# lehduong/Knowledge-Distillation-by-Replacing-Cheap-Conv

Measured on AMD Instinct MI355X. Metric: images/sec KD train step, DeepLabV3+(WRN38) student 1024x2048, higher is better.
Workload: dtype bf16; 1 GPU; KD train step (teacher fwd + student fwd + CE/KD/hint criteria + hint bwd + RAdam), DeepLabV3+(WRN-38) student P92, 1024x2048, 8 img/GPU, random init, teacher through the HIP engine; plan=P92, mode=A, arch=deeplab, hint_loss=mse, per_gpu_batch=8, global_batch=8, parallelism=dp1, teacher_backend=hip, ranks_seen=1

## Files before the change

include/kdcc.h:

```cpp
#ifndef KDCC_H
#define KDCC_H

#include <stddef.h>
#include <stdint.h>

#ifdef __cplusplus
extern "C" {
#endif

typedef void *kd_stream_t;

enum { KD_F32 = 0, KD_BF16 = 1 };
enum {
    KD_OK = 0,
    KD_ERR_INVALID = -1,
    KD_ERR_UNSUPPORTED = -2,
    KD_ERR_WORKSPACE = -3,
    KD_ERR_HIP = -4
};

int kd_version(void);
const char *kd_last_error(void);

typedef struct kd_conv_desc {
    int32_t dtype;
    int32_t N, H, W, Cin;
    int32_t Ho, Wo, Cout;
    int32_t kh, kw, stride, pad, dil;
    int32_t ldx;
} kd_conv_desc;

typedef struct kd_conv_epilogue {
    const void *res_pre;  int32_t ld_res_pre;
    const void *mask;     int32_t ld_mask;     const float *mask_scale;
    const void *res_post; int32_t ld_res_post;
    void *out_raw;        int32_t ld_raw;      int32_t raw_f32;
    void *out_act;        int32_t ld_act;      const float *act_scale; const float *act_shift; int32_t act_relu;
    float *bn_sums;
    const void *cls_w;    float *cls_out;      int32_t ld_cls;      int32_t ncls;
} kd_conv_epilogue;
int32_t kd_conv2d_cls_supported(const kd_conv_desc *d, const kd_conv_epilogue *ep);

int kd_conv2d_fwd(const kd_conv_desc *d, const void *x, const void *w_packed,
                  const kd_conv_epilogue *ep, kd_stream_t stream);
int32_t kd_conv2d_bn_sums_rows(const kd_conv_desc *d, const kd_conv_epilogue *ep);
size_t kd_bn_sums_finish_workspace(int32_t rows, int32_t C);
int kd_bn_sums_finish(const float *part, int32_t rows, int32_t C, float *s1, float *s2, void *workspace, size_t workspace_bytes,
                      kd_stream_t stream);

int32_t kd_conv1x1_dual_supported(const kd_conv_desc *d, int32_t Cin2, int32_t ldx2, const kd_conv_epilogue *ep);
int kd_conv1x1_dual_fwd(const kd_conv_desc *d, const void *x, const void *x2, int32_t Cin2, int32_t ldx2, const void *w_cat,
                        const kd_conv_epilogue *ep, kd_stream_t stream);

int kd_conv_set_persist_cus(int32_t n);

enum { KD_PACK_FWD = 0, KD_PACK_DGRAD = 1 };
int kd_pack_conv_weight(const float *src, void *dst, int32_t dtype, int32_t mode,
                        int32_t Cout, int32_t Cin, int32_t kh, int32_t kw, int32_t cin_pad,
                        kd_stream_t stream);

size_t kd_pw_wgrad_workspace(int32_t M, int32_t Cin, int32_t Cout);
int kd_pw_wgrad(int32_t dtype, int32_t M, int32_t Cin, int32_t Cout,
                const void *a, int32_t lda, const void *dy, int32_t ldy,
                float *dw, int32_t accumulate, void *workspace, size_t workspace_bytes,
                kd_stream_t stream);

size_t kd_conv2d_wgrad_workspace(const kd_conv_desc *d);
int kd_conv2d_wgrad(const kd_conv_desc *d, const void *x, const void *dy, int32_t ld_dy, float *dw,
                    int32_t accumulate, void *workspace, size_t workspace_bytes, kd_stream_t stream);

typedef struct kd_dw_desc {
    int32_t dtype;
    int32_t N, H, W, C;
    int32_t k, pad, dil;
    int32_t ldx, ldy;
} kd_dw_desc;
typedef struct kd_dw_epilogue {
    const void *res_pre;  int32_t ld_res_pre;
    const void *mask;     int32_t ld_mask;     const float *mask_scale;
    const void *res_post; int32_t ld_res_post;
} kd_dw_epilogue;
int kd_pack_dw_weight(const float *src , float *dst ,
                      int32_t C, int32_t k, int32_t flip, kd_stream_t stream);
int kd_dwconv_fwd(const kd_dw_desc *d, const void *x, const float *w_taps, const float *bias,
                  const kd_dw_epilogue *ep, void *y, kd_stream_t stream);
int kd_dwconv_fwd_sum(const kd_dw_desc *d, int32_t n, const void *const *xs, const float *const *w_taps, void *y,
                      kd_stream_t stream);
int kd_dwconv_fwd_fanout(const kd_dw_desc *d, int32_t n, const void *x, const float *const *w_taps, void *const *ys,
                         kd_stream_t stream);
size_t kd_dwconv_wgrad_workspace(const kd_dw_desc *d);
int kd_dwconv_wgrad(const kd_dw_desc *d, const void *x, const void *dy, int32_t ld_dy,
                    float *dw, int32_t accumulate, void *workspace, size_t workspace_bytes,
                    kd_stream_t stream);
size_t kd_dwconv_wgrad_multi_workspace(const kd_dw_desc *d, int32_t n);
int kd_dwconv_wgrad_multi(const kd_dw_desc *d, int32_t n, const void *x, const void *const *dys, int32_t ld_dy,
                          float *const *dws, int32_t accumulate, void *workspace, size_t workspace_bytes,
                          kd_stream_t stream);

int64_t kd_lattice_rows(int32_t N, int32_t H, int32_t W, int32_t dil);
int32_t kd_dwconv_lattice_ok(const kd_dw_desc *d, int32_t n);
int kd_lattice_rows_move(int32_t dtype, int32_t N, int32_t H, int32_t W, int32_t C, int32_t dil, void *img, int32_t ld_img,
                         void *rows, int32_t ld_rows, int32_t to_rows, kd_stream_t stream);
int kd_dwconv_fwd_fanout_lattice(const kd_dw_desc *d, int32_t n, const void *x, const float *const *w_taps, void *const *ys,
                                 kd_stream_t stream);
int kd_dwconv_fwd_sum_lattice(const kd_dw_desc *d, int32_t n, const void *const *xs, const float *const *w_taps, void *y,
                              kd_stream_t stream);
int kd_dwconv_wgrad_multi_lattice(const kd_dw_desc *d, int32_t n, const void *x, const void *const *dys, float *const *dws,
                                  int32_t accumulate, void *workspace, size_t workspace_bytes ,
                                  kd_stream_t stream);

int kd_stem_conv(int32_t dtype, const float *x_nchw, const float *w, void *y,
                 int32_t N, int32_t H, int32_t W, kd_stream_t stream);
int kd_stem_conv_pool(const float *x_nchw, const float *w, void *y_raw, void *y_act, const float *scale,
                      const float *shift, int32_t N, int32_t H, int32_t W, kd_stream_t stream);

int kd_maxpool3x3s2(int32_t dtype, const void *x, int32_t ldx, void *y_raw, int32_t ld_raw,
                    void *y_act, int32_t ld_act, const float *scale, const float *shift,
                    int32_t N, int32_t H, int32_t W, int32_t C, kd_stream_t stream);

int kd_upsample_bilinear_ac(const void *x, int32_t x_dtype, int32_t ldx, void *y, int32_t y_dtype, int32_t ldy,
                            int32_t N, int32_t H, int32_t W, int32_t C, int32_t Ho, int32_t Wo,
                            kd_stream_t stream);

int kd_upsample_bilinear(const void *x, int32_t x_dtype, int32_t ldx, void *y, int32_t y_dtype, int32_t ldy,
                         int32_t N, int32_t H, int32_t W, int32_t C, int32_t Ho, int32_t Wo, int32_t align_corners,
                         kd_stream_t stream);

size_t kd_aspp_image_pool_workspace(int32_t N, int32_t Cin, int32_t Cout);
int kd_aspp_image_pool(int32_t dtype, const void *x, int32_t ldx, const float *w, const float *scale,
                       const float *shift, void *y, int32_t ldy, int32_t N, int32_t H, int32_t W,
                       int32_t Cin, int32_t Cout, void *workspace, size_t workspace_bytes, kd_stream_t stream);
int kd_aspp_image_pool_sums(int32_t dtype, const float *part, const float *w, const float *scale, const float *shift, void *y,
                            int32_t ldy, int32_t N, int32_t H, int32_t W, int32_t Cin, int32_t Cout, void *workspace,
                            size_t workspace_bytes, kd_stream_t stream);

size_t kd_stem_wgrad_workspace(int32_t N, int32_t H, int32_t W);
int kd_stem_wgrad(int32_t dtype, const float *x_nchw, const void *dy, int32_t ld_dy, float *dw, int32_t N, int32_t H,
                  int32_t W, int32_t accumulate, void *workspace, size_t workspace_bytes, kd_stream_t stream);
size_t kd_maxpool3x3s2_bwd_workspace(int32_t N, int32_t H, int32_t W, int32_t C);
int kd_maxpool3x3s2_bwd(int32_t dtype, const void *x, int32_t ldx, const void *gy, int32_t ldgy, void *gx, int32_t ldgx,
                        int32_t N, int32_t H, int32_t W, int32_t C, void *workspace, size_t workspace_bytes,
                        kd_stream_t stream);
size_t kd_upsample_bilinear_ac_bwd_workspace(int32_t N, int32_t H, int32_t W, int32_t C, int32_t Ho, int32_t Wo);
int kd_upsample_bilinear_ac_bwd(const void *gy, int32_t gy_dtype, int32_t ldgy, void *gx, int32_t gx_dtype, int32_t ldgx,
                                int32_t N, int32_t H, int32_t W, int32_t C, int32_t Ho, int32_t Wo,
                                void *workspace, size_t workspace_bytes, kd_stream_t stream);
int kd_upsample_bilinear_bwd(const void *gy, int32_t gy_dtype, int32_t ldgy, void *gx, int32_t gx_dtype, int32_t ldgx,
                             int32_t N, int32_t H, int32_t W, int32_t C, int32_t Ho, int32_t Wo, int32_t align_corners,
// ... 219 lines not shown
```

knowledge-distillation-by-replacing-cheap-conv_amd/_lib.py:

```python
import ctypes as C
import os

_HERE = os.path.dirname(os.path.abspath(__file__))
_sel = os.environ.get("KDCC_LIB", "")
LIB_PATH = (os.path.join(_HERE, "libkdcc_hip_tuning.so") if _sel == "tuning" else _sel if _sel.endswith(".so")
            else os.path.join(_HERE, "libkdcc_hip.so"))


def build_tuning():
    import subprocess
    subprocess.check_call(["make", "-s", "-j", str(min(8, os.cpu_count() or 1)), "-C", os.path.join(_HERE, "csrc"), "TUNING=1"])

KD_F32, KD_BF16 = 0, 1
KD_PACK_FWD, KD_PACK_DGRAD = 0, 1
KD_ERR_UNSUPPORTED = -2
KD_OPT_SGD, KD_OPT_ADAM, KD_OPT_ADAMW_REF = 0, 1, 2
KD_OPT_FIRST, KD_OPT_NESTEROV, KD_OPT_AMSGRAD, KD_OPT_MAXIMIZE = 1, 2, 4, 8

c_int, c_i64, c_f, c_vp, c_sz = C.c_int32, C.c_int64, C.c_float, C.c_void_p, C.c_size_t


class ConvDesc(C.Structure):
    _fields_ = [(n, c_int) for n in ("dtype", "N", "H", "W", "Cin", "Ho", "Wo", "Cout", "kh", "kw", "stride", "pad",
                                     "dil", "ldx")]


class ConvEpilogue(C.Structure):
    _fields_ = [("res_pre", c_vp), ("ld_res_pre", c_int),
                ("mask", c_vp), ("ld_mask", c_int), ("mask_scale", c_vp),
                ("res_post", c_vp), ("ld_res_post", c_int),
                ("out_raw", c_vp), ("ld_raw", c_int), ("raw_f32", c_int),
                ("out_act", c_vp), ("ld_act", c_int), ("act_scale", c_vp), ("act_shift", c_vp), ("act_relu", c_int),
                ("bn_sums", c_vp),
                ("cls_w", c_vp), ("cls_out", c_vp), ("ld_cls", c_int), ("ncls", c_int)]


class DwDesc(C.Structure):
    _fields_ = [(n, c_int) for n in ("dtype", "N", "H", "W", "C", "k", "pad", "dil", "ldx", "ldy")]


class RadamTensor(C.Structure):
    _fields_ = [("p", c_vp), ("g", c_vp), ("exp_avg", c_vp), ("exp_avg_sq", c_vp), ("n", c_i64), ("step", c_int),
                ("lr", c_f), ("beta1", c_f), ("beta2", c_f), ("eps", c_f), ("weight_decay", c_f)]


class OptimTensor(C.Structure):
    _fields_ = [("p", c_vp), ("g", c_vp), ("state", c_vp * 3), ("n", c_i64), ("step", c_i64), ("flags", c_int), ("reserved", c_int),
                ("lr", C.c_double), ("weight_decay", C.c_double), ("eps", C.c_double), ("momentum", C.c_double),
                ("dampening", C.c_double), ("beta1", C.c_double), ("beta2", C.c_double), ("warmup", C.c_double)]


class DwEpilogue(C.Structure):
    _fields_ = [("res_pre", c_vp), ("ld_res_pre", c_int), ("mask", c_vp), ("ld_mask", c_int), ("mask_scale", c_vp),
                ("res_post", c_vp), ("ld_res_post", c_int)]


class DConvDesc(C.Structure):
    _fields_ = [(n, c_int) for n in ("N", "C", "H", "W", "K", "kh", "kw", "stride", "pad", "dil", "groups")]


class View3(C.Structure):
    _fields_ = [("ptr", c_vp), ("dtype", c_int), ("sN", c_i64), ("sC", c_i64), ("sP", c_i64)]


class HrView(C.Structure):
    _fields_ = [("ptr", c_vp), ("H", c_int), ("W", c_int), ("ld", c_int)]


KD_MULTI_MAX = 16


class MultiTargets(C.Structure):
    _fields_ = [("n", c_int), ("t", View3 * KD_MULTI_MAX), ("w", c_f * KD_MULTI_MAX)]


_P = C.POINTER
_SIGS = {
    "kd_version": (c_int, []),
    "kd_last_error": (C.c_char_p, []),
    "kd_conv2d_fwd": (c_int, [_P(ConvDesc), c_vp, c_vp, _P(ConvEpilogue), c_vp]),
    "kd_conv1x1_dual_supported": (c_int, [_P(ConvDesc), c_int, c_int, _P(ConvEpilogue)]),
    "kd_conv1x1_dual_fwd": (c_int, [_P(ConvDesc), c_vp, c_vp, c_int, c_int, c_vp, _P(ConvEpilogue), c_vp]),
    "kd_conv_set_persist_cus": (c_int, [c_int]),
    "kd_conv2d_bn_sums_rows": (c_int, [_P(ConvDesc), _P(ConvEpilogue)]),
    "kd_conv2d_cls_supported": (c_int, [_P(ConvDesc), _P(ConvEpilogue)]),
    "kd_bn_sums_finish_workspace": (c_sz, [c_int, c_int]),
    "kd_bn_sums_finish": (c_int, [c_vp, c_int, c_int, c_vp, c_vp, c_vp, c_sz, c_vp]),
    "kd_pack_conv_weight": (c_int, [c_vp, c_vp, c_int, c_int, c_int, c_int, c_int, c_int, c_int, c_vp]),
    "kd_pw_wgrad_workspace": (c_sz, [c_int, c_int, c_int]),
    "kd_pw_wgrad": (c_int, [c_int, c_int, c_int, c_int, c_vp, c_int, c_vp, c_int, c_vp, c_int, c_vp, c_sz, c_vp]),
    "kd_conv2d_wgrad_workspace": (c_sz, [_P(ConvDesc)]),
    "kd_conv2d_wgrad": (c_int, [_P(ConvDesc), c_vp, c_vp, c_int, c_vp, c_int, c_vp, c_sz, c_vp]),
    "kd_stem_wgrad_workspace": (c_sz, [c_int, c_int, c_int]),
    "kd_stem_wgrad": (c_int, [c_int, c_vp, c_vp, c_int, c_vp, c_int, c_int, c_int, c_int, c_vp, c_sz, c_vp]),
    "kd_maxpool3x3s2_bwd_workspace": (c_sz, [c_int, c_int, c_int, c_int]),
    "kd_maxpool3x3s2_bwd": (c_int, [c_int, c_vp, c_int, c_vp, c_int, c_vp, c_int, c_int, c_int, c_int, c_int, c_vp, c_sz, c_vp]),
    "kd_upsample_bilinear_ac_bwd_workspace": (c_sz, [c_int] * 6),
    "kd_upsample_bilinear_ac_bwd": (c_int, [c_vp, c_int, c_int, c_vp, c_int, c_int, c_int, c_int, c_int, c_int, c_int, c_int, c_vp,
                                            c_sz, c_vp]),
    "kd_zero_insert": (c_int, [c_int, c_vp, c_int, c_vp, c_int, c_int, c_int, c_int, c_int, c_int, c_int, c_int, c_vp]),
    "kd_relu_bn_bwd": (c_int, [c_int, c_vp, c_int, c_vp, c_int, c_vp, c_vp, c_int, c_vp, c_int, c_i64, c_int, c_vp]),
    "kd_channel_sums_workspace": (c_sz, [c_int, c_i64, c_int]),
    "kd_channel_sums": (c_int, [c_int, c_vp, c_int, c_vp, c_int, c_vp, c_int, c_int, c_i64, c_int, c_vp, c_vp, c_vp, c_sz, c_vp]),
    "kd_bn_eval_param_grads": (c_int, [c_vp, c_vp, c_vp, c_vp, c_vp, c_vp, c_vp, c_int, c_int, c_vp]),
    "kd_broadcast_add": (c_int, [c_int, c_vp, c_vp, c_int, c_int, c_i64, c_int, c_f, c_int, c_vp]),
    "kd_conv2d_direct_fwd": (c_int, [_P(DConvDesc), c_vp, c_vp, c_vp, c_vp, c_vp]),
    "kd_conv2d_direct_dgrad": (c_int, [_P(DConvDesc), c_vp, c_vp, c_vp, c_vp]),
    "kd_conv2d_direct_wgrad": (c_int, [_P(DConvDesc), c_vp, c_vp, c_vp, c_vp, c_int, c_vp]),
    "kd_bn2d_fwd": (c_int, [c_vp, c_vp, c_vp, c_vp, c_vp, c_vp, c_vp, c_vp, c_f, c_f, c_int, c_int, c_int, c_int, c_int, c_vp]),
    "kd_bn2d_bwd": (c_int, [c_vp, c_vp, c_vp, c_vp, c_vp, c_vp, c_vp, c_vp, c_vp, c_int, c_int, c_int, c_int, c_int, c_int, c_vp]),
    "kd_bn_nhwc_workspace": (c_sz, [c_i64, c_int]),
    "kd_bn_nhwc_fwd": (c_int, [c_vp, c_int, c_vp, c_int, c_i64, c_int, c_vp, c_vp, c_vp, c_vp, c_vp, c_vp, c_f, c_f, c_int, c_int,
                               c_vp, c_sz, c_vp]),
    "kd_bn_nhwc_bwd": (c_int, [c_vp, c_int, c_vp, c_int, c_vp, c_int, c_vp, c_int, c_vp, c_int, c_i64, c_int, c_vp, c_vp, c_vp, c_vp,
                               c_vp, c_int, c_int, c_int, c_vp, c_sz, c_vp]),
    "kd_bn_nhwc_stats": (c_int, [c_vp, c_int, c_i64, c_int, c_vp, c_vp, c_vp, c_f, c_vp, c_sz, c_vp]),
    "kd_bn_nhwc_apply": (c_int, [c_vp, c_int, c_vp, c_int, c_i64, c_int, c_vp, c_vp, c_vp, c_vp, c_vp, c_vp, c_vp, c_f, c_int, c_vp]),
    "kd_avgpool2x2_nhwc": (c_int, [c_vp, c_int, c_vp, c_int, c_int, c_int, c_int, c_int, c_vp]),
    "kd_avgpool2x2_nhwc_bwd": (c_int, [c_vp, c_int, c_vp, c_int, c_int, c_int, c_int, c_int, c_vp]),
    "kd_pack_dw_weight": (c_int, [c_vp, c_vp, c_int, c_int, c_int, c_vp]),
    "kd_dwconv_fwd": (c_int, [_P(DwDesc), c_vp, c_vp, c_vp, _P(DwEpilogue), c_vp, c_vp]),
    "kd_dwconv_fwd_sum": (c_int, [_P(DwDesc), c_int, c_vp, c_vp, c_vp, c_vp]),
    "kd_dwconv_fwd_fanout": (c_int, [_P(DwDesc), c_int, c_vp, c_vp, c_vp, c_vp]),
    "kd_dwconv_wgrad_workspace": (c_sz, [_P(DwDesc)]),
    "kd_dwconv_wgrad": (c_int, [_P(DwDesc), c_vp, c_vp, c_int, c_vp, c_int, c_vp, c_sz, c_vp]),
    "kd_dwconv_wgrad_multi_workspace": (c_sz, [_P(DwDesc), c_int]),
    "kd_dwconv_wgrad_multi": (c_int, [_P(DwDesc), c_int, c_vp, c_vp, c_int, c_vp, c_int, c_vp, c_sz, c_vp]),
    "kd_lattice_rows": (c_i64, [c_int, c_int, c_int, c_int]),
    "kd_dwconv_lattice_ok": (c_int, [_P(DwDesc), c_int]),
    "kd_lattice_rows_move": (c_int, [c_int, c_int, c_int, c_int, c_int, c_int, c_vp, c_int, c_vp, c_int, c_int, c_vp]),
    "kd_dwconv_fwd_fanout_lattice": (c_int, [_P(DwDesc), c_int, c_vp, c_vp, c_vp, c_vp]),
    "kd_dwconv_fwd_sum_lattice": (c_int, [_P(DwDesc), c_int, c_vp, c_vp, c_vp, c_vp]),
    "kd_dwconv_wgrad_multi_lattice": (c_int, [_P(DwDesc), c_int, c_vp, c_vp, c_vp, c_int, c_vp, c_sz, c_vp]),
    "kd_stem_conv": (c_int, [c_int, c_vp, c_vp, c_vp, c_int, c_int, c_int, c_vp]),
    "kd_scale_by_device_scalar": (c_int, [c_vp, c_int, c_i64, c_vp, c_vp]),
    "kd_pointwise_small": (c_int, [c_vp, c_int, c_vp, c_vp, c_vp, c_int, c_i64, c_int, c_int, c_vp]),
    "kd_conv3x3_small": (c_int, [c_vp, c_int, c_vp, c_vp, c_vp, c_int, c_vp, c_int, c_int, c_int, c_int, c_int, c_int, c_vp]),
    "kd_stem_conv_pool": (c_int, [c_vp, c_vp, c_vp, c_vp, c_vp, c_vp, c_int, c_int, c_int, c_vp]),
    "kd_maxpool3x3s2": (c_int, [c_int, c_vp, c_int, c_vp, c_int, c_vp, c_int, c_vp, c_vp, c_int, c_int, c_int, c_int, c_vp]),
    "kd_upsample_bilinear_ac": (c_int, [c_vp, c_int, c_int, c_vp, c_int, c_int, c_int, c_int, c_int, c_int, c_int, c_int, c_vp]),
    "kd_upsample_bilinear": (c_int, [c_vp, c_int, c_int, c_vp, c_int, c_int, c_int, c_int, c_int, c_int, c_int, c_int, c_int, c_vp]),
    "kd_gated_conv": (c_int, [c_int, c_vp, c_int, c_vp, c_int, c_vp, c_vp, c_int, c_i64, c_int, c_vp]),
    "kd_edge_attention": (c_int, [c_int, c_vp, c_int, c_vp, c_vp, c_vp, c_i64, c_vp]),
    "kd_edge_aspp": (c_int, [c_int, c_vp, c_int, c_int, c_vp, c_vp, c_vp, c_vp, c_int, c_int, c_int, c_int, c_int, c_vp]),
    "kd_canny_workspace": (c_sz, [c_int, c_int, c_int]),
    "kd_canny": (c_int, [c_vp, c_int, c_int, c_int, c_int, c_int, c_int, c_vp, c_vp, c_vp, c_sz, c_vp]),
    "kd_canny_continue": (c_int, [c_int, c_int, c_int, c_int, c_vp, c_vp, c_vp, c_sz, c_vp]),
    "kd_aspp_image_pool_workspace": (c_sz, [c_int, c_int, c_int]),
    "kd_aspp_image_pool": (c_int, [c_int, c_vp, c_int, c_vp, c_vp, c_vp, c_vp, c_int, c_int, c_int, c_int, c_int, c_int,
                                   c_vp, c_sz, c_vp]),
    "kd_aspp_image_pool_sums": (c_int, [c_int, c_vp, c_vp, c_vp, c_vp, c_vp, c_int, c_int, c_int, c_int, c_int, c_int, c_vp, c_sz, c_vp]),
    "kd_bn_fold": (c_int, [c_vp, c_vp, c_vp, c_vp, c_f, c_vp, c_vp, c_int, c_vp]),
    "kd_copy_cast": (c_int, [c_vp, c_int, c_i64, c_i64, c_i64, c_vp, c_int, c_i64, c_i64, c_i64, c_int, c_int, c_i64, c_vp]),
    "kd_loss_workspace": (c_sz, [c_int, c_int, c_i64]),
    "kd_kldiv": (c_int, [_P(View3), _P(View3), c_f, c_int, c_int, c_i64, c_vp, _P(View3), c_f, c_vp, c_sz, c_vp]),
    "kd_hint_mse": (c_int, [_P(View3), _P(View3), c_f, c_int, c_int, c_i64, c_vp, _P(View3), c_f, c_vp, c_sz, c_vp]),
    "kd_weighted_hint_mse": (c_int, [_P(View3), _P(View3), c_vp, c_int, c_int, c_int, c_i64, c_vp, _P(View3), c_f, c_vp,
                                     c_sz, c_vp]),
    "kd_ce2d": (c_int, [_P(View3), c_vp, c_int, c_int, c_int, c_i64, c_vp, c_vp, c_sz, c_vp]),
    "kd_ce2d_up": (c_int, [c_vp, c_vp, c_int, c_int, c_int, c_int, c_int, c_int, c_int, c_int, c_vp, c_vp, c_sz, c_vp]),
    "kd_kldiv_up": (c_int, [c_vp, c_vp, c_f, c_int, c_int, c_int, c_int, c_int, c_int, c_int, c_vp, c_vp, c_sz, c_vp]),
    "kd_logit_metrics_up": (c_int, [c_vp, c_vp, c_vp, c_int, c_int, c_int, c_int, c_int, c_int, c_int, c_int, c_vp, c_vp, c_vp, c_int,
                                    c_vp, c_sz, c_vp]),
    "kd_ce2d_grad": (c_int, [_P(View3), c_vp, c_int, c_int, c_int, c_i64, _P(View3), c_f, c_vp, c_sz, c_vp]),
    "kd_ce2d_weighted": (c_int, [_P(View3), c_vp, c_vp, c_int, c_int, c_int, c_int, c_i64, c_vp, c_vp, c_sz, c_vp]),
    "kd_ce2d_weighted_grad": (c_int, [_P(View3), c_vp, c_vp, c_int, c_int, c_int, c_int, c_i64, _P(View3), c_f, c_vp, c_sz, c_vp]),
    "kd_jsdiv": (c_int, [_P(View3), _P(View3), c_f, c_int, c_int, c_i64, c_vp, _P(View3), c_f, c_vp, c_sz, c_vp]),
    "kd_jsdiv_up": (c_int, [c_vp, c_vp, c_f, c_int, c_int, c_int, c_int, c_int, c_int, c_int, c_vp, c_vp, c_sz, c_vp]),
    "kd_ensemble_kldiv": (c_int, [_P(View3), _P(View3), c_int, c_int, c_i64, c_vp, _P(View3), c_f, c_vp, c_sz, c_vp]),
    "kd_kldiv_multi": (c_int, [_P(View3), _P(MultiTargets), c_f, c_vp, c_int, c_f, c_f, c_int, c_int, c_i64, c_vp, _P(View3), c_vp, c_sz, c_vp]),
    "kd_softmax_mean": (c_int, [_P(MultiTargets), c_f, c_int, c_int, c_i64, _P(View3), c_vp]),
    "kd_focal": (c_int, [_P(View3), c_vp, c_vp, c_f, c_int, c_int, c_int, c_int, c_i64, c_vp, c_vp, c_vp, c_vp, c_vp, c_sz, c_vp]),
    "kd_focal_grad": (c_int, [_P(View3), c_vp, c_vp, c_f, c_int, c_int, c_int, c_int, c_i64, c_vp, c_vp, c_vp, c_vp, _P(View3), c_vp]),
# ... 94 lines not shown
```

knowledge-distillation-by-replacing-cheap-conv_amd/engine.py:

```python
import itertools
import os

import torch
from torch import nn

from . import ops
from ._lib import KD_PACK_DGRAD, KD_PACK_FWD
from .lazy import LazyLogits
from .models.students.transform_blocks import DepthwiseSeparableBlock, GateLayer, RandomMask2d
from .models.wider_resnet import IdentityResidualBlock

_SMALL_CONV = os.environ.get("KDCC_SMALL_CONV", "1") != "0"
_SPLIT_DEC_DGRAD = os.environ.get("KDCC_SPLIT_DEC_DGRAD", "1") != "0"
_STEM_POOL = os.environ.get("KDCC_STEM_POOL", "1") != "0"
_DW_SUM = os.environ.get("KDCC_DW_SUM", "1") != "0"
_CONV_DUAL = os.environ.get("KDCC_CONV_DUAL", "1") != "0"
_FUSE_BN_SUMS = os.environ.get("KDCC_FUSE_BN_SUMS", "1") != "0"
_FUSE_GAP = os.environ.get("KDCC_FUSE_GAP", "1") != "0"


class EngineError(RuntimeError):
    pass


_FOLD_SERIAL = itertools.count(1)


def _is_trainable(mod):
    return any(p.requires_grad for p in mod.parameters())


def _bn_of(bn_seq):
    return bn_seq[0] if isinstance(bn_seq, nn.Sequential) else bn_seq


def _gate_split(mod):
    if isinstance(mod, nn.Sequential) and len(mod) == 2 and isinstance(mod[1], GateLayer):
        return mod[0], mod[1]
    return mod, None


def _is_masked(mod):
    return (isinstance(mod, nn.Sequential) and len(mod) == 3 and isinstance(mod[0], nn.Conv2d) and isinstance(mod[1], RandomMask2d)
            and isinstance(mod[2], nn.Conv2d))


def _act_gate(bn_seq):
    if isinstance(bn_seq, nn.Sequential) and len(bn_seq) > 1:
        return _gate_split(bn_seq[1])[1]
    return None


class _Site:

    def __init__(self, name, mod):
        mod, self.gate = _gate_split(mod)
        self.name, self.mod = name, mod
        self.cheap = isinstance(mod, DepthwiseSeparableBlock)
        self.masked = _is_masked(mod)
        if self.masked:
            self._init_masked(name, mod)
            return
        if self.cheap and self.gate is not None:
            raise EngineError(f"{name}: a gate behind a cheap-conv block is not supported (gates rank the TEACHER's filters)")
        if not self.cheap and not isinstance(mod, nn.Conv2d):
            raise EngineError(f"{name}: unsupported module {type(mod).__name__} in the student graph")
        conv = mod.pointwise_conv if self.cheap else mod
        self.cout = conv.out_channels
        self.cin = (mod.separable_conv if self.cheap else conv).in_channels
        if self.cheap:
            self.k, self.pad, self.dil = mod.geometry
            self.stride = 1
            if mod.separable_conv.bias is not None or mod.pointwise_conv.bias is not None:
                raise EngineError(f"{name}: biased cheap conv inside the fused graph is not supported")
        else:
            if conv.bias is not None or conv.groups != 1:
                raise EngineError(f"{name}: only bias-free dense convs are supported")
            self.k, self.pad, self.dil, self.stride = conv.kernel_size[0], conv.padding[0], conv.dilation[0], conv.stride[0]
        self.trainable = _is_trainable(mod) or (self.gate is not None and self.gate.weight.requires_grad)

    def _init_masked(self, name, mod):
        conv, mask, pw = mod[0], mod[1], mod[2]
        if self.gate is not None:
            raise EngineError(f"{name}: a gate behind a masked site is not supported")
        if conv.bias is not None or conv.groups != 1 or _is_trainable(conv):
            raise EngineError(f"{name}: the conv in front of a RandomMask2d must be a frozen, bias-free dense conv")
        if pw.bias is not None or pw.kernel_size != (1, 1) or pw.stride != (1, 1) or pw.padding != (0, 0) or pw.groups != 1 or \
                pw.in_channels != conv.out_channels or mask.in_channels != conv.out_channels:
            raise EngineError(f"{name}: the conv behind a RandomMask2d must be a bias-free 1x1 over the masked channels")
        self.cin, self.cout = conv.in_channels, pw.out_channels
        self.k, self.pad, self.dil, self.stride = conv.kernel_size[0], conv.padding[0], conv.dilation[0], conv.stride[0]
        self.trainable = pw.weight.requires_grad


class StudentEngine:
    def __init__(self, net, dtype=torch.bfloat16):
        self.net = net
        self.dtype = dtype
        self.hint_names = []
        self._pack = {}
# ... 940 lines not shown
        if gate is not None:
            s2 = s2 / gate.weight.detach().float()
            if gate.weight.requires_grad and grads is not None:
                gbuf = self._grad_like(gate.weight)
                gbuf.copy_(s2)
                grads[gate.weight] = gbuf
                self._grad_done(gate.weight)
        self.probe_grads[name] = s2

    def _conv_wgrad(self, conv, a_in, g, grads, cin=None, cin_rot=0, gate=None):
        w = conv.weight
        if not w.requires_grad:
            return
        if cin is not None and cin != a_in.shape[3]:
            a_in = a_in[..., :cin]
        gw = self._grad_like(w)
        if cin_rot:
            tmp = torch.empty_like(gw)
            ops.conv2d_wgrad(a_in, g, tmp, conv.stride[0], conv.padding[0], conv.dilation[0])
            k = w.shape[1] - cin_rot
            gw[:, cin_rot:].copy_(tmp[:, :k])
            gw[:, :cin_rot].copy_(tmp[:, k:])
        else:
            ops.conv2d_wgrad(a_in, g, gw, conv.stride[0], conv.padding[0], conv.dilation[0])
        if gate is not None:
            gw.mul_(gate.weight.detach().float().view(-1, 1, 1, 1))
        grads[w] = gw
        self._grad_done(w)

    def _wants_bn_sums(self, bn_seq, gate=None):
        bn = _bn_of(bn_seq)
        return bn.weight.requires_grad or bn.bias.requires_grad or (gate is not None and gate.weight.requires_grad)

    def _bn_param_grads(self, bn_seq, g_x, act, grads, sub=None, gate=None, sums=None):
        bn = _bn_of(bn_seq)
        want_gate = gate is not None and gate.weight.requires_grad
        if not (bn.weight.requires_grad or bn.bias.requires_grad or want_gate):
            return
        scale, _ = self._bn_fold(bn_seq)
        s1, s2 = sums if sums is not None else ops.channel_sums(g_x, sub=sub, a=act)
        if gate is not None:
            gv = gate.weight.detach().float()
            if want_gate:
                gbuf = self._grad_like(gate.weight)
                gbuf.copy_(torch.where(scale != 0, s2 / (scale * gv * gv), torch.zeros_like(s2)))
                grads[gate.weight] = gbuf
                self._grad_done(gate.weight)
            s2 = s2 / gv
        if bn.weight.requires_grad or bn.bias.requires_grad:
            self._bn_grads_from_sums(bn, scale, s1, s2, grads)

    def _bn_grads_from_sums(self, bn, scale, s1, s2, grads):
        dg, db = self._grad_like(bn.weight), self._grad_like(bn.bias)
        ops.bn_eval_param_grads(s1.contiguous(), s2.contiguous(), scale, bn.weight.detach().float().contiguous(),
                                bn.bias.detach().float().contiguous(), dg, db)
        for p, gbuf in ((bn.weight, dg), (bn.bias, db)):
            if p.requires_grad:
                grads[p] = gbuf
                self._grad_done(p)

    def _dense_dgrad(self, site, g, in_hw=None, **ep):
        conv = site.mod
        N, H, W, _ = g.shape
        if site.stride != 1:
            if in_hw is None:
                raise EngineError(f"{site.name}: strided input gradient needs the input size")
            g = ops.zero_insert(g, site.stride, in_hw)
            H, W = in_hw
        out = self._new(N, H, W, conv.in_channels)
        ops.conv2d(g, self._w_dgrad(conv, gate=site.gate), 1, site.dil * (site.k - 1) - site.pad, site.dil, out_raw=out, **ep)
        return out

    def _cheap_bwd(self, site, a_in, mid, g, grads, need_in, defer=None, **ep):
        dw, pw = site.mod.separable_conv, site.mod.pointwise_conv
        if pw.weight.requires_grad:
            gw = self._grad_like(pw.weight)
            ops.pw_wgrad(mid, g, gw)
            grads[pw.weight] = gw
            self._grad_done(pw.weight)
        if not (dw.weight.requires_grad or need_in):
            return None
        N, H, W, _ = g.shape
        g_mid = self._new(N, H, W, pw.in_channels)
        ops.conv2d(g, self._w_dgrad(pw), out_raw=g_mid)
        if dw.weight.requires_grad and defer is None:
            gw = self._grad_like(dw.weight)
            ops.dwconv_wgrad(a_in, g_mid, gw, site.k, site.pad, site.dil)
            grads[dw.weight] = gw
            self._grad_done(dw.weight)
        if defer is not None:
            defer.append((g_mid, self._w_dw(dw, True) if need_in else None, site, dw.weight if dw.weight.requires_grad else None))
            return None
        if not need_in:
            return None
        return ops.dwconv(g_mid, self._w_dw(dw, True), site.k, site.dil * (site.k - 1) - site.pad, site.dil, **ep)

    def _site_bwd(self, site, a_in, mid, g, grads, need_in, **ep):
        if site.cheap:
            return self._cheap_bwd(site, a_in, mid, g, grads, need_in, **ep)
        if site.masked:
            return self._masked_bwd(site, mid, g, grads, need_in)
        self._conv_wgrad(site.mod, a_in, g, grads, gate=site.gate)
        if not need_in:
            return None
        return self._dense_dgrad(site, g, in_hw=(a_in.shape[1], a_in.shape[2]), **ep)

    def _block_bwd(self, bi, rec, g_out, g_site_hint, grads):
        blk, sites = rec["blk"], rec["sites"]
        bns = {n: m for n, m in blk.convs.named_children() if n.startswith("bn")}
        g = g_out
        for i in range(len(sites) - 1, -1, -1):
            site, a_in, need_in = sites[i], rec["a_in"][i], rec["rg_a"][i]
            g_in = None
            bn_seq = bns[f"bn{i + 1}"] if i > 0 else blk.bn1
            act_gate = _act_gate(bn_seq) if i > 0 else None
            if g is not None and i in rec.get("probe", {}):
                self._probe(site.name, g, *rec["probe"][i], gate=site.gate, grads=grads)
            if g is not None and (need_in or site.trainable):
                sc, _ = self._act_fold(bn_seq, act_gate)
                ep = dict(mask=a_in, mask_scale=sc)
                sub = None
                if i > 0:
                    sub = g_site_hint.get((bi, i - 1))
                    ep["res_post"] = sub
                elif g_out is not None:
                    if rec["proj"]:
                        psite = _Site(f"{rec['name']}.proj_conv", blk.proj_conv)
                        self._conv_wgrad(blk.proj_conv, a_in, g_out, grads)
                        dual_bwd = (need_in and site.k == 1 and site.stride == 1 and g_out.is_contiguous() and g.is_contiguous() and
                                    self._dual_ok(g.shape, site.cout, g_out.shape[3], site.cin, 1, site.mod, blk.proj_conv, site))
                        if need_in and not dual_bwd:
                            ep["res_pre"] = self._dense_dgrad(psite, g_out, in_hw=(a_in.shape[1], a_in.shape[2]))
                    elif rec["rg_in"]:
                        sub = g_out
                        ep["res_post"] = g_out
                fused = []
                if _FUSE_BN_SUMS and need_in and not site.cheap and self._wants_bn_sums(bn_seq, act_gate):
                    ep["bn_sums"] = fused
                if i == 0 and g_out is not None and rec["proj"] and dual_bwd:
                    self._conv_wgrad(site.mod, a_in, g, grads, gate=site.gate)
                    g_in = self._new(g.shape[0], g.shape[1], g.shape[2], site.cin)
                    try:
                        ops.conv2d(g, self._w_cat(site.mod, blk.proj_conv, "dgrad"), out_raw=g_in, x2=g_out, **ep)
                    except ops.DualUnsupported:
                        if ep.get("bn_sums") is not None:
                            del ep["bn_sums"][:]
                        ep["res_pre"] = self._dense_dgrad(psite, g_out, in_hw=(a_in.shape[1], a_in.shape[2]))
                        g_in = self._dense_dgrad(site, g, in_hw=(a_in.shape[1], a_in.shape[2]), **ep)
                else:
                    g_in = self._site_bwd(site, a_in, rec["mid"][i], g, grads, need_in, **ep)
                if g_in is not None:
                    self._bn_param_grads(bn_seq, g_in, a_in, grads, sub=sub, gate=act_gate, sums=fused[0] if fused else None)
            elif i == 0 and g is None and g_out is not None:
                if rec["proj"]:
                    self._conv_wgrad(blk.proj_conv, a_in, g_out, grads)
                    if need_in:
                        psite = _Site(f"{rec['name']}.proj_conv", blk.proj_conv)
                        sc, _ = self._bn_fold(blk.bn1)
                        g_in = self._dense_dgrad(psite, g_out, in_hw=(a_in.shape[1], a_in.shape[2]), mask=a_in, mask_scale=sc)
                        self._bn_param_grads(blk.bn1, g_in, a_in, grads)
                elif rec["rg_in"]:
                    g_in = g_out
            if i > 0:
                if g_in is None:
                    g_in = g_site_hint.get((bi, i - 1)) if rec["rg_a"][i] else None
                g = g_in
            else:
# ... 282 lines not shown
```

knowledge-distillation-by-replacing-cheap-conv_amd/ops.py:

```python
import ctypes as C
import os

import torch

from . import _lib
from ._lib import (KD_BF16, KD_F32, KD_PACK_DGRAD, KD_PACK_FWD, ConvDesc, ConvEpilogue, DConvDesc, DwDesc, DwEpilogue, MultiTargets, View3,
                   check)


PROFILER = None


def _prof_start():
    if PROFILER is None:
        return None
    e0 = torch.cuda.Event(enable_timing=True)
    e0.record()
    return e0


def _prof_stop(e0, family, work, label, kernel=None):
    if e0 is None or PROFILER is None:
        return
    e1 = torch.cuda.Event(enable_timing=True)
# ... 155 lines not shown
        check(_lib.lib().kd_conv1x1_dual_fwd(C.byref(d), _ptr(x), _ptr(x2), Cin2, ld2, _ptr(w_packed), C.byref(ep), stream_ptr()), "kd_conv1x1_dual_fwd")
    else:
        check(_lib.lib().kd_conv2d_fwd(C.byref(d), _ptr(x), _ptr(w_packed), C.byref(ep), stream_ptr()), "kd_conv2d_fwd")
    if out_rows > 0:
        out_sums.append(opart)
    if prof is not None:
        e1 = torch.cuda.Event(enable_timing=True)
        e1.record()
        epi = "".join(c for c, t in (("p", res_pre), ("m", mask), ("q", res_post), ("r", out_raw), ("a", out_act), ("c", cls_out)) if t is not None)
        prof.append(("conv_igemm", 2.0 * N * Ho * Wo * (algo_cout or Cout) * kh * kw * (algo_cin or (Cin + Cin2)), e0, e1,
                     f"{kh}x{kw} s{stride} d{dil} {H}x{W} {Cin}{'+%d' % Cin2 if Cin2 else ''}->{Cout} [{epi}{'s' if sums_rows or out_rows else ''}]", _lib.last_kernel()))
    if sums_rows > 0:
        s12 = torch.empty((2, Cout), dtype=torch.float32, device=x.device)
        need = _lib.lib().kd_bn_sums_finish_workspace(sums_rows, Cout)
        ws = _ws(need, x.device) if need else None
        check(_lib.lib().kd_bn_sums_finish(_ptr(part), sums_rows, Cout, _ptr(s12[0]), _ptr(s12[1]), _ptr(ws), need, stream_ptr()),
              "kd_bn_sums_finish")
        bn_sums.append((s12[0], s12[1]))
    return out_raw, out_act


def conv_cls_ok(x, Cout, k=3, dil=1):
    if not x.is_cuda or x.dtype != torch.bfloat16 or os.environ.get("KDCC_FUSE_CLS", "1") == "0":
        return False
    N, H, W, Cin = x.shape
    d = ConvDesc(dt_of(x), N, H, W, Cin, H, W, Cout, k, k, 1, dil * (k // 2), dil, nhwc_ld(x))
    ep = ConvEpilogue()
    ep.cls_w, ep.cls_out, ep.ld_cls, ep.ncls = C.c_void_p(256), C.c_void_p(256), 32, 19
    return bool(_lib.lib().kd_conv2d_cls_supported(C.byref(d), C.byref(ep)))


def conv1x1_dual_ok(x, x2, Cout, operands=0):
    if x2 is None or not x.is_cuda or x.dtype != torch.bfloat16 or x2.dtype != x.dtype or tuple(x2.shape[:3]) != tuple(x.shape[:3]):
        return False
    N, H, W, Cin = x.shape
    d = ConvDesc(dt_of(x), N, H, W, Cin, H, W, Cout, 1, 1, 1, 0, 1, nhwc_ld(x))
    ep = ConvEpilogue()
    some = C.c_void_p(x.data_ptr())
    if operands >= 1:
        ep.mask, ep.ld_mask = some, Cout
    if operands >= 2:
        ep.res_post, ep.ld_res_post = some, Cout
    if operands >= 3:
        ep.res_pre, ep.ld_res_pre = some, Cout
    ep.out_raw, ep.ld_raw = some, Cout
    return bool(_lib.lib().kd_conv1x1_dual_supported(C.byref(d), x2.shape[3], nhwc_ld(x2), C.byref(ep)))


def conv1x1_dual_ok_dims(N, H, W, Cin, Cin2, Cout, dtype, operands=0):
    if dtype != torch.bfloat16:
        return False
    d = ConvDesc(KD_BF16, N, H, W, Cin, H, W, Cout, 1, 1, 1, 0, 1, Cin)
    ep = ConvEpilogue()
    if operands >= 1:
        ep.mask, ep.ld_mask = C.c_void_p(256), Cout
    if operands >= 2:
        ep.res_post, ep.ld_res_post = C.c_void_p(256), Cout
    if operands >= 3:
        ep.res_pre, ep.ld_res_pre = C.c_void_p(256), Cout
    ep.out_raw, ep.ld_raw = C.c_void_p(256), Cout
    return bool(_lib.lib().kd_conv1x1_dual_supported(C.byref(d), Cin2, Cin2, C.byref(ep)))


def pw_wgrad(a, dy, dw, accumulate=False, workspace=None):
    _need_cuda(a, dy, dw)
    N, H, W, Cin = a.shape
    Cout = dy.shape[3]
    if tuple(dy.shape[:3]) != (N, H, W) or a.dtype != dy.dtype:
        raise ValueError("pw_wgrad: a / dy mismatch")
    if dw.dtype != torch.float32 or dw.numel() != Cout * Cin or not dw.is_contiguous():
        raise ValueError("pw_wgrad: dw must be contiguous fp32 (Cout,Cin,1,1)")
    M = N * H * W
    need = _lib.lib().kd_pw_wgrad_workspace(M, Cin, Cout)
    if workspace is None or workspace.numel() * workspace.element_size() < need:
        workspace = torch.empty(need, dtype=torch.uint8, device=a.device)
    e0 = _prof_start()
    check(_lib.lib().kd_pw_wgrad(dt_of(a), M, Cin, Cout, _ptr(a), nhwc_ld(a), _ptr(dy), nhwc_ld(dy), _ptr(dw),
                                 int(accumulate), _ptr(workspace), workspace.numel() * workspace.element_size(),
                                 stream_ptr()), "kd_pw_wgrad")
    _prof_stop(e0, "pw_wgrad", 2.0 * M * Cin * Cout, f"pw wgrad {H}x{W} {Cin}->{Cout}")
    return dw


def conv2d_wgrad(x, dy, dw, stride=1, pad=0, dil=1, accumulate=False, workspace=None):
    _need_cuda(x, dy, dw)
    N, H, W, Cin = x.shape
    Cout, Cin_w, kh, kw = dw.shape
    Ho, Wo = conv_out_size(H, kh, stride, pad, dil), conv_out_size(W, kw, stride, pad, dil)
    if Cin_w != Cin or tuple(dy.shape) != (N, Ho, Wo, Cout) or dy.dtype != x.dtype:
        raise ValueError(f"conv2d_wgrad: x {tuple(x.shape)} / dy {tuple(dy.shape)} / dw {tuple(dw.shape)} mismatch")
    if dw.dtype != torch.float32 or not dw.is_contiguous():
        raise ValueError("conv2d_wgrad: dw must be contiguous fp32 (Cout,Cin,kh,kw)")
    d = ConvDesc(dt_of(x), N, H, W, Cin, Ho, Wo, Cout, kh, kw, stride, pad, dil, nhwc_ld(x))
    need = _lib.lib().kd_conv2d_wgrad_workspace(C.byref(d))
    if workspace is None or workspace.numel() * workspace.element_size() < need:
        workspace = torch.empty(need, dtype=torch.uint8, device=x.device)
    prof = PROFILER
    if prof is not None:
        e0 = torch.cuda.Event(enable_timing=True)
        e0.record()
    check(_lib.lib().kd_conv2d_wgrad(C.byref(d), _ptr(x), _ptr(dy), nhwc_ld(dy), _ptr(dw), int(accumulate), _ptr(workspace),
                                     workspace.numel() * workspace.element_size(), stream_ptr()), "kd_conv2d_wgrad")
    if prof is not None:
        e1 = torch.cuda.Event(enable_timing=True)
        e1.record()
        prof.append(("conv_wgrad", 2.0 * N * Ho * Wo * Cout * kh * kw * Cin, e0, e1,
                     f"wgrad {kh}x{kw} s{stride} d{dil} {H}x{W} {Cin}->{Cout}", _lib.last_kernel()))
    return dw


def pack_dw_weight(w, flip=False):
    _need_cuda(w)
    w = w.detach().contiguous().float()
    Cc, one, k, k2 = w.shape
    if one != 1 or k != k2:
        raise ValueError("pack_dw_weight: expected (C,1,k,k)")
    out = torch.empty((k * k, Cc), dtype=torch.float32, device=w.device)
    check(_lib.lib().kd_pack_dw_weight(_ptr(w), _ptr(out), Cc, k, int(flip), stream_ptr()), "kd_pack_dw_weight")
    return out


def _dw_desc(x, k, pad, dil, y=None):
    N, H, W, Cc = x.shape
    return DwDesc(dt_of(x), N, H, W, Cc, k, pad, dil, nhwc_ld(x), nhwc_ld(y) if y is not None else Cc)


def _dw_taps(who, w_taps, k, Cc):
    for w in w_taps:
        if tuple(w.shape) != (k * k, Cc) or w.dtype != torch.float32 or not w.is_contiguous():
            raise ValueError(f"{who}: w_taps must be contiguous fp32 [k*k][C]")


def _dw_grads(who, dws, k, Cc):
    for dw in dws:
        if dw.dtype != torch.float32 or dw.numel() != Cc * k * k or not dw.is_contiguous():
            raise ValueError(f"{who}: dw must be contiguous fp32 (C,1,k,k)")


def _dw_out(who, out, shape, like):
    if out is None:
        out = torch.empty(shape, dtype=like.dtype, device=like.device)
    if tuple(out.shape) != tuple(shape) or out.dtype != like.dtype:
        raise ValueError(f"{who}: bad output view")
    return out


def _ptrs(ts):
    return (C.c_void_p * len(ts))(*[_ptr(t) for t in ts])


def _lattice_t(ts):
    return [t.t for t in ts]


def dwconv(x, w_taps, k, pad, dil, bias=None, out=None, res_pre=None, mask=None, mask_scale=None, res_post=None):
    _need_cuda(x, w_taps, bias, out, res_pre, mask, mask_scale, res_post)
    if bias is not None and (bias.dtype != torch.float32 or not bias.is_contiguous()):
        bias = bias.detach().float().contiguous()
    N, H, W, Cc = x.shape
    _dw_taps("dwconv", [w_taps], k, Cc)
    out = _dw_out("dwconv", out, (N, H, W, Cc), x)
    d = _dw_desc(x, k, pad, dil, out)
    ep = None
    if res_pre is not None or mask is not None or res_post is not None:
        ep = DwEpilogue()
        for name, t in (("res_pre", res_pre), ("mask", mask), ("res_post", res_post)):
# ... 1444 lines not shown
```

Before: 46.16 images/sec.

## Add dedicated pointwise dgrad kernel for cheap-conv backward pass

```diff
diff --git a/include/kdcc.h b/include/kdcc.h
--- a/include/kdcc.h
+++ b/include/kdcc.h
@@ -64,6 +64,11 @@
                 const void *a, int32_t lda, const void *dy, int32_t ldy,
                 float *dw, int32_t accumulate, void *workspace, size_t workspace_bytes,
                 kd_stream_t stream);
+
+int32_t kd_pw_dgrad_supported(int32_t dtype, int64_t M, int32_t K, int32_t N, const void *g, int32_t ldg, const void *w,
+                              const void *out, int32_t ldo);
+int kd_pw_dgrad(int32_t dtype, int64_t M, int32_t K, int32_t N, const void *g, int32_t ldg, const void *w, void *out,
+                int32_t ldo, kd_stream_t stream);
 
 size_t kd_conv2d_wgrad_workspace(const kd_conv_desc *d);
 int kd_conv2d_wgrad(const kd_conv_desc *d, const void *x, const void *dy, int32_t ld_dy, float *dw,
diff --git a/knowledge-distillation-by-replacing-cheap-conv_amd/_lib.py b/knowledge-distillation-by-replacing-cheap-conv_amd/_lib.py
--- a/knowledge-distillation-by-replacing-cheap-conv_amd/_lib.py
+++ b/knowledge-distillation-by-replacing-cheap-conv_amd/_lib.py
@@ -89,6 +89,8 @@
     "kd_pack_conv_weight": (c_int, [c_vp, c_vp, c_int, c_int, c_int, c_int, c_int, c_int, c_int, c_vp]),
     "kd_pw_wgrad_workspace": (c_sz, [c_int, c_int, c_int]),
     "kd_pw_wgrad": (c_int, [c_int, c_int, c_int, c_int, c_vp, c_int, c_vp, c_int, c_vp, c_int, c_vp, c_sz, c_vp]),
+    "kd_pw_dgrad_supported": (c_int, [c_int, c_i64, c_int, c_int, c_vp, c_int, c_vp, c_vp, c_int]),
+    "kd_pw_dgrad": (c_int, [c_int, c_i64, c_int, c_int, c_vp, c_int, c_vp, c_vp, c_int, c_vp]),
     "kd_conv2d_wgrad_workspace": (c_sz, [_P(ConvDesc)]),
     "kd_conv2d_wgrad": (c_int, [_P(ConvDesc), c_vp, c_vp, c_int, c_vp, c_int, c_vp, c_sz, c_vp]),
     "kd_stem_wgrad_workspace": (c_sz, [c_int, c_int, c_int]),
diff --git a/knowledge-distillation-by-replacing-cheap-conv_amd/csrc/pw_dgrad.hip b/knowledge-distillation-by-replacing-cheap-conv_amd/csrc/pw_dgrad.hip
--- /dev/null
+++ b/knowledge-distillation-by-replacing-cheap-conv_amd/csrc/pw_dgrad.hip
@@ -0,0 +1,157 @@
+#include "igemm_core.h"
+#include "pw_dgrad_select.h"
+
+namespace {
+struct PwDgradParams {
+    const bf16_t *g, *w;
+    bf16_t *out;
+    long long M;
+    int N, ldg, ldo;
+};
+
+template <int KS>
+__global__ __launch_bounds__(512) void pw_dgrad_kernel(const PwDgradParams p)
+{
+    constexpr int K = 32 * KS, ROWB = 64 * KS, CPR = 4 * KS, SLAB = PW_DGRAD_BN * ROWB;
+    constexpr int SW = KS % 4 == 0 ? 15 : KS % 2 == 0 ? 7 : 3;
+    constexpr int NP = (CPR + 7) / 8;
+    constexpr int NST = 8;
+    static_assert(2 * SLAB <= 64 * 1024, "two weight slabs");
+    __shared__ __attribute__((aligned(16))) char lds[2 * SLAB + 8 * 2048];
+
+    const int tid = threadIdx.x, lane = tid & 63;
+    const int wv = __builtin_amdgcn_readfirstlane(tid >> 6);
+    const int frow = lane & 15, fq = lane >> 4;
+
+    int woff[NP];
+#pragma unroll
+    for (int t = 0; t < NP; ++t) {
+        const int pi = KS % 2 == 0 ? wv * NP + t : t * 8 + wv;
+        const int q = pi * 64 + lane, rho = q / CPR, c = (q % CPR) ^ (rho & SW);
+        const int chan = (rho & 32) + (((rho & 15) >> 2) << 3) + (((rho >> 4) & 1) << 2) + (rho & 3);
+        woff[t] = chan * K + c * 8;
+    }
+    auto stage = [&](int slab, int buf) {
+        const bf16_t *wb = p.w + (size_t)slab * (PW_DGRAD_BN * K);
+        char *lb = lds + buf * SLAB;
+        if constexpr (KS == 8) {
+            glds16_x4(wb + woff[0], (const char *)(wb + woff[1]) - 1024, (const char *)(wb + woff[2]) - 2048,
+                      (const char *)(wb + woff[3]) - 3072, lb + wv * 4096);
+        } else {
+#pragma unroll
+            for (int t = 0; t < NP; ++t) {
+                const int pi = KS % 2 == 0 ? wv * NP + t : t * 8 + wv;
+                if (pi < CPR) glds16(wb + woff[t], lb + pi * 1024);
+            }
+        }
+        __builtin_amdgcn_sched_barrier(0);
+    };
+    stage(0, 0);
+
+    uint4 a[4][KS];
+    bf16_t *orow0[4], *orow1[4];
+    const int r0 = lane >> 3, cc = lane & 7;
+    const long long m_wave = (long long)blockIdx.x * PW_DGRAD_BM + wv * 64;
+#pragma unroll
+    for (int i = 0; i < 4; ++i) {
+        long long pm = m_wave + i * 16 + frow;
+        pm = pm < p.M ? pm : p.M - 1;
+        const bf16_t *gr = p.g + pm * p.ldg + fq * 8;
+#pragma unroll
+        for (int ks = 0; ks < KS; ++ks) a[i][ks] = *(const uint4 *)(gr + ks * 32);
+        long long p0 = m_wave + i * 16 + r0, p1 = p0 + 8;
+        p0 = p0 < p.M ? p0 : p.M - 1;
+        p1 = p1 < p.M ? p1 : p.M - 1;
+        orow0[i] = p.out + p0 * p.ldo + cc * 8;
+        orow1[i] = p.out + p1 * p.ldo + cc * 8;
+    }
+    asm volatile("s_waitcnt vmcnt(0)" ::: "memory");
+    __builtin_amdgcn_s_barrier();
+
+    const int nslab = p.N / PW_DGRAD_BN;
+    const int swz = frow & SW, wsw = (frow >> 1) & 7;
+    char *patch = lds + 2 * SLAB + wv * 2048;
+#pragma unroll 1
+    for (int c = 0; c < nslab; ++c) {
+        if (c + 1 < nslab) stage(c + 1, (c + 1) & 1);
+        const char *sb = lds + (c & 1) * SLAB + frow * ROWB;
+        f32x4_t acc[4][4];
+#pragma unroll
+        for (int i = 0; i < 4; ++i)
+#pragma unroll
+            for (int j = 0; j < 4; ++j) acc[i][j] = (f32x4_t){0.f, 0.f, 0.f, 0.f};
+#pragma unroll
+        for (int s = 0; s < 2; ++s)
+#pragma unroll
+            for (int ks = 0; ks < KS; ++ks) {
+                uint4 b[2];
+#pragma unroll
+                for (int h = 0; h < 2; ++h) b[h] = *(const uint4 *)(sb + (2 * s + h) * 16 * ROWB + (((ks * 4 + fq) ^ swz) << 4));
+#pragma unroll
+                for (int i = 0; i < 4; ++i)
+#pragma unroll
+                    for (int h = 0; h < 2; ++h) Mma<bf16_t>::run(b[h], a[i][ks], acc[i][2 * s + h]);
+            }
+#pragma unroll
+        for (int i = 0; i < 4; ++i) {
+            uint4 v[2];
+#pragma unroll
+            for (int s = 0; s < 2; ++s)
+                v[s] = make_uint4(pack_bf16x2(acc[i][2 * s][0], acc[i][2 * s][1]), pack_bf16x2(acc[i][2 * s][2], acc[i][2 * s][3]),
+                                  pack_bf16x2(acc[i][2 * s + 1][0], acc[i][2 * s + 1][1]), pack_bf16x2(acc[i][2 * s + 1][2], acc[i][2 * s + 1][3]));
+            *(uint4 *)(patch + frow * 128 + ((fq ^ wsw) << 4)) = v[0];
+            *(uint4 *)(patch + frow * 128 + (((4 + fq) ^ wsw) << 4)) = v[1];
+            const uint4 s0 = *(const uint4 *)(patch + r0 * 128 + ((cc ^ ((r0 >> 1) & 7)) << 4));
+            const uint4 s1 = *(const uint4 *)(patch + (r0 + 8) * 128 + ((cc ^ (((r0 + 8) >> 1) & 7)) << 4));
+            *(uint4 *)(orow0[i] + c * PW_DGRAD_BN) = s0;
+            *(uint4 *)(orow1[i] + c * PW_DGRAD_BN) = s1;
+        }
+        asm volatile("s_waitcnt vmcnt(%0) lgkmcnt(0)" ::"n"(NST) : "memory");
+        __builtin_amdgcn_s_barrier();
+    }
+}
+
+PwDgradProblem pw_dgrad_problem(int32_t dtype, int64_t M, int32_t K, int32_t N, const void *g, int32_t ldg, const void *w,
+                                       const void *out, int32_t ldo)
+{
+    PwDgradProblem q;
+    q.dtype = dtype; q.M = M; q.K = K; q.N = N; q.g = g; q.w = w; q.out = out; q.ldg = ldg; q.ldo = ldo;
+    return q;
+}
+
+}
+
+extern "C" int32_t kd_pw_dgrad_supported(int32_t dtype, int64_t M, int32_t K, int32_t N, const void *g, int32_t ldg, const void *w,
+                                         const void *out, int32_t ldo)
+{
+    return g && w && out && pw_dgrad_ok(pw_dgrad_problem(dtype, M, K, N, g, ldg, w, out, ldo));
+}
+
+extern "C" int kd_pw_dgrad(int32_t dtype, int64_t M, int32_t K, int32_t N, const void *g, int32_t ldg, const void *w, void *out,
+                           int32_t ldo, kd_stream_t stream)
+{
+    KD_REQUIRE(g && w && out, KD_ERR_INVALID, "kd_pw_dgrad: null argument");
+    KD_REQUIRE(dtype == KD_F32 || dtype == KD_BF16, KD_ERR_INVALID, "kd_pw_dgrad: bad dtype");
+    KD_REQUIRE(M > 0 && K > 0 && N > 0 && ldg >= K && ldo >= N, KD_ERR_INVALID, "kd_pw_dgrad: bad shape");
+    KD_REQUIRE(pw_dgrad_ok(pw_dgrad_problem(dtype, M, K, N, g, ldg, w, out, ldo)), KD_ERR_UNSUPPORTED,
+               "kd_pw_dgrad: needs bf16, K %% 32 == 0 and <= %d, N %% %d == 0, 16-byte aligned views (M=%lld K=%d N=%d ldg=%d ldo=%d): "
+               "run kd_conv2d_fwd", PW_DGRAD_MAXK, PW_DGRAD_BN, (long long)M, K, N, ldg, ldo);
+    PwDgradParams p;
+    p.g = (const bf16_t *)g; p.w = (const bf16_t *)w; p.out = (bf16_t *)out;
+    p.M = M; p.N = N; p.ldg = ldg; p.ldo = ldo;
+    const dim3 grid(pw_dgrad_grid(M));
+    hipStream_t s = (hipStream_t)stream;
+    KD_NOTE_KERNEL("pw_dgrad_kernel");
+    switch (K / 32) {
+    case 1: hipLaunchKernelGGL(pw_dgrad_kernel<1>, grid, dim3(512), 0, s, p); break;
+    case 2: hipLaunchKernelGGL(pw_dgrad_kernel<2>, grid, dim3(512), 0, s, p); break;
+    case 3: hipLaunchKernelGGL(pw_dgrad_kernel<3>, grid, dim3(512), 0, s, p); break;
+    case 4: hipLaunchKernelGGL(pw_dgrad_kernel<4>, grid, dim3(512), 0, s, p); break;
+    case 5: hipLaunchKernelGGL(pw_dgrad_kernel<5>, grid, dim3(512), 0, s, p); break;
+    case 6: hipLaunchKernelGGL(pw_dgrad_kernel<6>, grid, dim3(512), 0, s, p); break;
+    case 7: hipLaunchKernelGGL(pw_dgrad_kernel<7>, grid, dim3(512), 0, s, p); break;
+    default: hipLaunchKernelGGL(pw_dgrad_kernel<8>, grid, dim3(512), 0, s, p); break;
+    }
+    KD_CHECK_LAUNCH("kd_pw_dgrad");
+    return KD_OK;
+}
diff --git a/knowledge-distillation-by-replacing-cheap-conv_amd/csrc/pw_dgrad_select.h b/knowledge-distillation-by-replacing-cheap-conv_amd/csrc/pw_dgrad_select.h
--- /dev/null
+++ b/knowledge-distillation-by-replacing-cheap-conv_amd/csrc/pw_dgrad_select.h
@@ -0,0 +1,30 @@
+#pragma once
+#include <stdint.h>
+
+#include "../../include/kdcc.h"
+
+constexpr int PW_DGRAD_BM = 512;
+constexpr int PW_DGRAD_BN = 64;
+constexpr int PW_DGRAD_MAXK = 256;
+
+struct PwDgradProblem {
+    int32_t dtype;
+    int64_t M;
+    int32_t K, N;
+    const void *g, *w, *out;
+    int32_t ldg, ldo;
+};
+
+static inline bool pw_dgrad_aligned16(const void *p) { return (reinterpret_cast<uintptr_t>(p) & 15u) == 0; }
+
+static inline bool pw_dgrad_ok(const PwDgradProblem &q)
+{
+    if (q.dtype != KD_BF16) return false;
+    if (q.M <= 0 || q.M >= (1ll << 31)) return false;
+    if (q.K <= 0 || q.K % 32 != 0 || q.K > PW_DGRAD_MAXK) return false;
+    if (q.N <= 0 || q.N % PW_DGRAD_BN != 0) return false;
+    if (q.ldg < q.K || q.ldo < q.N || q.ldg % 8 != 0 || q.ldo % 8 != 0) return false;
+    return pw_dgrad_aligned16(q.g) && pw_dgrad_aligned16(q.w) && pw_dgrad_aligned16(q.out);
+}
+
+static inline unsigned pw_dgrad_grid(int64_t M) { return (unsigned)((M + PW_DGRAD_BM - 1) / PW_DGRAD_BM); }
diff --git a/knowledge-distillation-by-replacing-cheap-conv_amd/engine.py b/knowledge-distillation-by-replacing-cheap-conv_amd/engine.py
--- a/knowledge-distillation-by-replacing-cheap-conv_amd/engine.py
+++ b/knowledge-distillation-by-replacing-cheap-conv_amd/engine.py
@@ -16,6 +16,7 @@
 _DW_SUM = os.environ.get("KDCC_DW_SUM", "1") != "0"
 _CONV_DUAL = os.environ.get("KDCC_CONV_DUAL", "1") != "0"
 _FUSE_BN_SUMS = os.environ.get("KDCC_FUSE_BN_SUMS", "1") != "0"
+_PW_DGRAD = os.environ.get("KDCC_PW_DGRAD", "1") != "0"
 _FUSE_GAP = os.environ.get("KDCC_FUSE_GAP", "1") != "0"
 
 
@@ -1122,7 +1123,11 @@
             return None
         N, H, W, _ = g.shape
         g_mid = self._new(N, H, W, pw.in_channels)
-        ops.conv2d(g, self._w_dgrad(pw), out_raw=g_mid)
+        w_d = self._w_dgrad(pw)
+        if _PW_DGRAD and ops.pw_dgrad_ok(g, w_d, g_mid):
+            ops.pw_dgrad(g, w_d, g_mid)
+        else:
+            ops.conv2d(g, w_d, out_raw=g_mid)
         if dw.weight.requires_grad and defer is None:
             gw = self._grad_like(dw.weight)
             ops.dwconv_wgrad(a_in, g_mid, gw, site.k, site.pad, site.dil)
diff --git a/knowledge-distillation-by-replacing-cheap-conv_amd/ops.py b/knowledge-distillation-by-replacing-cheap-conv_amd/ops.py
--- a/knowledge-distillation-by-replacing-cheap-conv_amd/ops.py
+++ b/knowledge-distillation-by-replacing-cheap-conv_amd/ops.py
@@ -261,6 +261,38 @@
     return dw
 
 
+class PwDgradUnsupported(_lib.KdccError):
+    """pw_dgrad() on a problem kd_pw_dgrad does not take (pw_dgrad_ok() says which): run conv2d on the same operands."""
+
+
+def _pw_dgrad_args(g, w_packed, out):
+    _need_cuda(g, w_packed, out)
+    N, H, W, K = g.shape
+    Cn, kh, kw, Kw = w_packed.shape
+    if (kh, kw) != (1, 1) or Kw != K or tuple(out.shape) != (N, H, W, Cn):
+        raise ValueError(f"pw_dgrad: g {tuple(g.shape)} / packed weight {tuple(w_packed.shape)} / out {tuple(out.shape)} mismatch")
+    if w_packed.dtype != g.dtype or out.dtype != g.dtype or not w_packed.is_contiguous():
+        raise ValueError("pw_dgrad: the packed weight must be contiguous, and it and out of the gradient's dtype")
+    return dt_of(g), N * H * W, K, Cn, _ptr(g), nhwc_ld(g), _ptr(w_packed), _ptr(out), nhwc_ld(out)
+
+
+def pw_dgrad_ok(g, w_packed, out):
+    return bool(_lib.lib().kd_pw_dgrad_supported(*_pw_dgrad_args(g, w_packed, out)))
+
+
+def pw_dgrad(g, w_packed, out):
+    args = _pw_dgrad_args(g, w_packed, out)
+    _, M, K, Cn = args[:4]
+    H, W = g.shape[1:3]
+    e0 = _prof_start()
+    rc = _lib.lib().kd_pw_dgrad(*args, stream_ptr())
+    if rc == _lib.KD_ERR_UNSUPPORTED:
+        raise PwDgradUnsupported(f"pw_dgrad: {_lib.lib().kd_last_error().decode()}")
+    check(rc, "kd_pw_dgrad")
+    _prof_stop(e0, "conv_igemm", 2.0 * M * Cn * K, f"1x1 s1 d1 {H}x{W} {K}->{Cn} [r]")
+    return out
+
+
 def conv2d_wgrad(x, dy, dw, stride=1, pad=0, dil=1, accumulate=False, workspace=None):
     _need_cuda(x, dy, dw)
     N, H, W, Cin = x.shape
```

Result: no change. 46.28 images/sec (median of 6 runs) (+0.3%).
